# ShijieZhou-UCLA/feature-3dgs

Hardware: NVIDIA H100
Metric: views/sec fwd+bwd @1M Gaussians/1080p/feat_dim=128 (higher is better)
Workload: dtype f32

## Files before the change

### feature-3dgs_b200/csrc/composite_common.cuh

```cuda
#pragma once
#include <initializer_list>

#include "kernels.h"

namespace f3dgs {

constexpr int kBlocksPerTile = 8;
constexpr int kProducerWarp = 0;
constexpr int kAlphaWarp0 = 4;
constexpr int kAlphaWarps = kBlocksPerTile;
constexpr int kFeatWarp0 = kAlphaWarp0 + kAlphaWarps;
constexpr int kRegsProducer = 40;
constexpr int kStageEntries = 32;
constexpr int kStages = 6;
constexpr int kWSlots = 2;
constexpr int kDoneSlots = 8;

template <int CH, typename TF = float>
struct alignas(128) Stage {
    TF feat[CH > 0 ? kStageEntries : 1][CH > 0 ? CH : 4];
    float4 rec0[kStageEntries];
    float4 rec1[kStageEntries];
    float4 rec2[kStageEntries];
    uint32_t listpos[kStageEntries];
    uint32_t gid[kStageEntries];
    uint32_t n;
    uint32_t last;
    uint32_t first;
    int32_t work;
    uint32_t done_slot;
};

struct alignas(128) WSlot {
    float w[kStageEntries][32];
    uint32_t pm[kStageEntries];
    uint32_t km;
    uint32_t last;
    uint32_t first;
    int32_t work;
};

template <int CH, typename TF = float, int WB = kBlocksPerTile, int WJ = kWSlots>
struct alignas(128) RingV2 {
    using Feat = TF;
    static constexpr int kWB = WB, kWJ = WJ;
    Stage<CH, TF> stage[kStages];
    WSlot ws[WB][WJ];
    uint64_t full[kStages];
    uint64_t empty[kStages];
    uint64_t listed[kStages];
    uint64_t wfull[WB][WJ];
    uint64_t wempty[WB][WJ];
    uint32_t done_mask[kDoneSlots];
};

using RingSlim = RingV2<0, float, 1, 1>;

static_assert(sizeof(RingV2<0>) == 81664 && sizeof(RingSlim) == 16128, "ring layout changed");
static_assert(sizeof(RingV2<32>) == 106240 && sizeof(RingV2<64>) == 130816 && sizeof(RingV2<128>) == 179968,
              "ring layout changed");
static_assert(sizeof(RingV2<32, __half>) == 93952 && sizeof(RingV2<64, __half>) == 106240 &&
                  sizeof(RingV2<128, __half>) == 130816,
              "ring layout changed");

__device__ __forceinline__ int block_x0(int tile_x, int b) { return tile_x * 16 + (b & 1) * 8; }
__device__ __forceinline__ int block_y0(int tile_y, int b) { return tile_y * 16 + (b >> 1) * 4; }
__device__ __forceinline__ int slot_px(int p) { return ((p >> 2) & 3) * 2 + (p & 1); }
__device__ __forceinline__ int slot_py(int p) { return (p >> 4) * 2 + ((p >> 1) & 1); }

template <int NQ>
__device__ __forceinline__ float& tile_px(float2 (&t)[NQ][2][4], int qi, int i, int c) {
    return (i & 1) ? t[qi][i >> 1][c].y : t[qi][i >> 1][c].x;
}
template <int NQ>
__device__ __forceinline__ float& tile_run_px(float2 (&t)[NQ][2][4], int y, int half, int k, int c) {
    return tile_px(t, ((y >> 1) * 4 + half * 2 + (k >> 1)) % NQ, (y & 1) * 2 + (k & 1), c);
}
template <int NQ>
__device__ __forceinline__ float4 tile_run(float2 (&t)[NQ][2][4], int y, int half, int c) {
    return make_float4(tile_run_px(t, y, half, 0, c), tile_run_px(t, y, half, 1, c), tile_run_px(t, y, half, 2, c),
                       tile_run_px(t, y, half, 3, c));
}
template <int NQ>
__device__ __forceinline__ void set_tile_run(float2 (&t)[NQ][2][4], int y, int half, int c, float4 v) {
    tile_run_px(t, y, half, 0, c) = v.x;
    tile_run_px(t, y, half, 1, c) = v.y;
    tile_run_px(t, y, half, 2, c) = v.z;
    tile_run_px(t, y, half, 3, c) = v.w;
}

template <int G, int NQ, typename T, class Row, class Run, class Px>
__device__ __forceinline__ void for_tile_pixels(T* plane, int bx0, int by0, int W, int H, int grp, bool rows, bool runs,
                                                Row row, Run run, Px px) {
    if (G == 1 && rows && bx0 + 8 <= W) {
#pragma unroll
        for (int y = 0; y < 4; y++) {
            const int yy = by0 + y;
            if (yy >= H) continue;
            row(plane + (size_t)yy * W + bx0, y);
        }
    } else if (G == 1 && runs) {
#pragma unroll
        for (int y = 0; y < 4; y++) {
            const int yy = by0 + y;
            if (yy >= H) continue;
#pragma unroll
            for (int half = 0; half < 2; half++) {
                const int xx = bx0 + half * 4;
                if (xx >= W) continue;
                run(plane + (size_t)yy * W + xx, y, half);
            }
        }
    } else {
#pragma unroll
        for (int qi = 0; qi < NQ; qi++) {
            const int q = qi * G + grp;
#pragma unroll
            for (int i = 0; i < 4; i++) {
                const int xx = bx0 + (q & 3) * 2 + (i & 1), yy = by0 + (q >> 2) * 2 + (i >> 1);
                if (xx < W && yy < H) px(plane + (size_t)yy * W + xx, qi, i);
            }
        }
    }
}

__device__ __forceinline__ float4 to_float4(float4 v) { return v; }
__device__ __forceinline__ float4 to_float4(uint2 v) {
    const float2 a = __half22float2(*reinterpret_cast<const __half2*>(&v.x));
    const float2 b = __half22float2(*reinterpret_cast<const __half2*>(&v.y));
    return make_float4(a.x, a.y, b.x, b.y);
}

__device__ __forceinline__ size_t list_begin(uint32_t begin, uint32_t end, int b) {
    return kBlocksPerTile * (size_t)begin + (size_t)b * (end - begin);
}

struct SplatAlpha {
    float dx, dy, G, alpha;
};
__device__ __forceinline__ SplatAlpha splat_alpha(const float4 r0, const float4 r1, float pxf, float pyf, bool valid) {
    SplatAlpha s;
    s.dx = r0.x - pxf;
    s.dy = r0.y - pyf;
    const float power = -0.5f * (r1.x * s.dx * s.dx + r1.z * s.dy * s.dy) - r1.y * s.dx * s.dy;
    s.G = expf(power);
    const float av = fminf(0.99f, r1.w * s.G);
    s.alpha = (valid && !(power > 0.0f) && !(av < 1.0f / 255.0f)) ? av : 0.f;
    return s;
}

__device__ __forceinline__ bool footprint_hits_rect(const float4 r0, const float4 r1, float x0, float x1, float y0,
                                                    float y1) {
    const bool box = (r0.x + r0.z >= x0) && (r0.x - r0.z <= x1) && (r0.y + r0.w >= y0) && (r0.y - r0.w <= y1);
    if (!box) return false;
    const float dxl = r0.x - x1, dxh = r0.x - x0, dyl = r0.y - y1, dyh = r0.y - y0;
    if (r0.z > 1.0e30f || (dxl <= 0.f && dxh >= 0.f && dyl <= 0.f && dyh >= 0.f)) return true;
    const float a = r1.x, b = r1.y, c = r1.z;
    const float tau = 2.02f * __logf(255.0f * r1.w) + 0.02f;
    const float nb_ia = -b * rcp_approx(a), nb_ic = -b * rcp_approx(c);
    float q = 3.0e38f;
#pragma unroll
    for (int k = 0; k < 2; k++) {
        const float ex_ = k ? dxh : dxl;
        const float ty = fminf(fmaxf(nb_ic * ex_, dyl), dyh);
        q = fminf(q, a * ex_ * ex_ + (2.f * b * ex_ + c * ty) * ty);
        const float ey_ = k ? dyh : dyl;
        const float tx = fminf(fmaxf(nb_ia * ey_, dxl), dxh);
        q = fminf(q, c * ey_ * ey_ + (2.f * b * ey_ + a * tx) * tx);
    }
    return q <= tau;
}

template <int N>
__device__ __forceinline__ void reg_dec() {
    asm volatile("setmaxnreg.dec.sync.aligned.u32 %0;" ::"n"(N));
}
template <int N>
__device__ __forceinline__ void reg_inc() {
    asm volatile("setmaxnreg.inc.sync.aligned.u32 %0;" ::"n"(N));
}

template <int CH, typename RING>
__device__ __forceinline__ void ring_init(RING& ring, int n_stage_consumers, int n_full_arrivals = 1) {
    if (threadIdx.x == 0) {
        for (int s = 0; s < kStages; s++) {
            mbar_init(&ring.full[s], n_full_arrivals);
            mbar_init(&ring.empty[s], n_stage_consumers);
            mbar_init(&ring.listed[s], 1);
        }
        for (int b = 0; b < RING::kWB; b++)
            for (int j = 0; j < RING::kWJ; j++) {
                mbar_init(&ring.wfull[b][j], 1);
                mbar_init(&ring.wempty[b][j], 1);
            }
        for (int i = 0; i < kDoneSlots; i++) ring.done_mask[i] = 0;
        mbar_fence_init();
    }
    if (CH > 0) {
        float4* p = reinterpret_cast<float4*>(&ring.stage[0]);
        const int n16 = (int)(sizeof(ring.stage) / 16);
        for (int i = threadIdx.x; i < n16; i += blockDim.x) p[i] = make_float4(0.f, 0.f, 0.f, 0.f);
        asm volatile("fence.proxy.async.shared::cta;" ::: "memory");
    }
}

struct ProducerArgs {
    const uint2* ranges;
    const uint32_t* point_list;
    const SplatRec* rec;
    const void* features;
    const uint32_t* n_contrib;
    int* work_counter;
    int W, H, C;
    int tiles_x, num_tiles, chunks;
    int use_bulk;
};

inline ProducerArgs producer_args(const ViewParams& vp, const uint2* ranges, const uint32_t* point_list,
                                  const SplatRec* rec, const uint32_t* n_contrib, int* work_counter) {
    return ProducerArgs{ranges, point_list, rec, nullptr, n_contrib, work_counter, vp.W, vp.H, 0, (int)vp.grid_x,
                        (int)(vp.grid_x * vp.grid_y), 1, 0};
}

inline int channel_chunk(int C) { return C <= 32 ? 32 : (C <= 64 ? 64 : 128); }

template <auto... K>
cudaError_t device_sms(int& sms, size_t smem) {
    static std::atomic<int> sms_of_device[64];
    int dev = 0;
    cudaGetDevice(&dev);
    if (dev < 0 || dev >= 64) return cudaErrorInvalidDevice;
    if (sms_of_device[dev].load() == 0) {
        for (const void* k : std::initializer_list<const void*>{reinterpret_cast<const void*>(K)...}) {
            const cudaError_t e = cudaFuncSetAttribute(k, cudaFuncAttributeMaxDynamicSharedMemorySize, (int)smem);
            if (e != cudaSuccess) return e;
        }
        int n = 0;
        cudaDeviceGetAttribute(&n, cudaDevAttrMultiProcessorCount, dev);
        sms_of_device[dev].store(n > 0 ? n : 132);
    }
    sms = sms_of_device[dev].load();
    return cudaSuccess;
}

template <int CH, bool REVERSE, typename RING = RingV2<CH>>
__device__ __forceinline__ void producer_loop(RING& ring, const ProducerArgs& pa) {
    using TF = typename RING::Feat;
    constexpr bool COPYWARP = CH > 0;
    const int lane = threadIdx.x & 31;
    int s = 0;
    uint32_t empty_parity = 1;
    mbar_wait(&ring.empty[0], empty_parity);

    uint32_t seq = 0;
    auto publish = [&](uint32_t n, uint32_t last, uint32_t first, int work) {
        __syncwarp();
        if (lane == 0) {
            Stage<CH, TF>& st = ring.stage[s];
            st.done_slot = seq % kDoneSlots;
            st.n = n;
            st.last = last;
            st.first = first;
            st.work = work;
            mbar_arrive(&ring.full[s]);
            if (COPYWARP) mbar_arrive(&ring.listed[s]);
        }
        __syncwarp();
    };
    auto advance = [&]() {
        s++;
        if (s == kStages) {
            s = 0;
            empty_parity ^= 1;
        }
        mbar_wait_sleep(&ring.empty[s], empty_parity, 64);
    };

    const int num_work = pa.num_tiles * pa.chunks;
    int pending = 0;
    if (lane == 0) pending = atomicAdd(pa.work_counter, 1);
    for (;;) {
        const int work = __shfl_sync(0xffffffffu, pending, 0);
        if (lane == 0 && work < num_work) pending = atomicAdd(pa.work_counter, 1);
        if (work >= num_work) {
            publish(0, 1, 1, -1);
            break;
        }
        const int tile = work / pa.chunks, chunk = work - tile * pa.chunks;
        const int tile_x = tile % pa.tiles_x, tile_y = tile / pa.tiles_x;
        const uint2 range = pa.ranges[tile];
        const uint32_t range_begin = range.x;
        uint32_t walk_count = range.y - range.x;
        if (REVERSE) {
            uint32_t tmax = 0;
            const int yy = tile_y * 16 + (lane >> 1), xb = tile_x * 16 + (lane & 1) * 8;
            if (yy < pa.H)
                for (int i = 0; i < 8; i++)
                    if (xb + i < pa.W) tmax = max(tmax, pa.n_contrib[(size_t)yy * pa.W + xb + i]);
#pragma unroll
            for (int o = 16; o > 0; o >>= 1) tmax = max(tmax, __shfl_xor_sync(0xffffffffu, tmax, o));
            walk_count = min(walk_count, tmax);
        }
        const float tx0 = (float)(tile_x * 16), ty0 = (float)(tile_y * 16), tx1 = tx0 + 15.f, ty1 = ty0 + 15.f;
        const int chunk_off = chunk * CH;
        const int row_floats = (CH > 0 && pa.features != nullptr) ? min(CH, pa.C - chunk_off) : 0;
        seq++;
        uint32_t* done = &ring.done_mask[seq % kDoneSlots];
        if (lane == 0) *reinterpret_cast<volatile uint32_t*>(done) = 0;
        __syncwarp();

        auto list_index = [&](uint32_t i) -> uint32_t {
            return REVERSE ? (range_begin + walk_count - 1 - i) : (range_begin + i);
        };
        auto store_entry = [&](uint32_t slot, uint32_t gid, uint32_t lpos, float4 r0, float4 r1, float4 r2) {
            Stage<CH, TF>& st = ring.stage[s];
            st.rec0[slot] = r0;
            st.rec1[slot] = r1;
            st.rec2[slot] = r2;
            st.listpos[slot] = lpos;
            st.gid[slot] = gid;
            if (CH > 0 && row_floats > 0) {
                const TF* src = static_cast<const TF*>(pa.features) + (size_t)gid * pa.C + chunk_off;
                if (!pa.use_bulk)
                    for (int c = 0; c < row_floats; c++) st.feat[slot][c] = __ldg(src + c);
            }
        };

        uint32_t fill = 0, first = 1;
        const uint32_t nchunks = (walk_count + 31) / 32;
        uint32_t id_cur = 0, id_nxt = 0;
        float4 a0, a1, a2;
        a0 = a1 = a2 = make_float4(0.f, 0.f, 0.f, 0.f);
        if (nchunks > 0) {
            if (lane < walk_count) id_cur = pa.point_list[list_index(lane)];
            if (32 + lane < walk_count) id_nxt = pa.point_list[list_index(32 + lane)];
            if (lane < walk_count) {
                const float4* r = reinterpret_cast<const float4*>(pa.rec + id_cur);
                a0 = __ldg(r); a1 = __ldg(r + 1); a2 = __ldg(r + 2);
            }
        }
        for (uint32_t c = 0; c < nchunks; c++) {
            if (*reinterpret_cast<volatile uint32_t*>(done) == (1u << kBlocksPerTile) - 1u) break;
            float4 b0, b1, b2;
            b0 = b1 = b2 = make_float4(0.f, 0.f, 0.f, 0.f);
            const uint32_t i1 = (c + 1) * 32 + lane, i2 = (c + 2) * 32 + lane;
            uint32_t id_nn = 0;
            if (i1 < walk_count) {
                const float4* r = reinterpret_cast<const float4*>(pa.rec + id_nxt);
                b0 = __ldg(r); b1 = __ldg(r + 1); b2 = __ldg(r + 2);
            }
            if (i2 < walk_count) id_nn = pa.point_list[list_index(i2)];

            const uint32_t i0 = c * 32 + lane;
            const bool valid = i0 < walk_count;
            const bool keep = valid && footprint_hits_rect(a0, a1, tx0, tx1, ty0, ty1);
            const uint32_t m = __ballot_sync(0xffffffffu, keep);
            const uint32_t cnt = __popc(m);
            const uint32_t rank = __popc(m & ((1u << lane) - 1u));
            const uint32_t lpos = list_index(i0) - range_begin + 1;
            const uint32_t room = kStageEntries - fill;
            if (keep && rank < room) store_entry(fill + rank, id_cur, lpos, a0, a1, a2);
            if (cnt >= room) {
                publish(kStageEntries, 0, first, work);
                first = 0;
                advance();
                if (keep && rank >= room) store_entry(rank - room, id_cur, lpos, a0, a1, a2);
                fill = cnt - room;
            } else {
                fill += cnt;
            }
            a0 = b0; a1 = b1; a2 = b2;
            id_cur = id_nxt;
            id_nxt = id_nn;
        }
        publish(fill, 1, first, work);
        advance();
    }
}

template <int CH, typename TF>
__device__ __forceinline__ void copy_loop(RingV2<CH, TF>& ring, const ProducerArgs& pa) {
    const int lane = threadIdx.x & 31;
    int s = 0;
    uint32_t parity = 0;
    for (;;) {
        mbar_wait(&ring.listed[s], parity);
        Stage<CH, TF>& st = ring.stage[s];
        const uint32_t n = st.n;
        const int work = st.work;
        if (work < 0) {
            if (lane == 0) mbar_arrive(&ring.full[s]);
            break;
        }
        const int chunk_off = (work % pa.chunks) * CH;
        const uint32_t row_bytes = (uint32_t)min(CH, pa.C - chunk_off) * (uint32_t)sizeof(TF);
        if (pa.use_bulk && n > 0) {
            if (lane == 0) mbar_arrive_expect_tx(&ring.full[s], n * row_bytes);
            __syncwarp();
            if (lane < n)
                bulk_g2s(&st.feat[lane][0],
                         static_cast<const TF*>(pa.features) + (size_t)st.gid[lane] * pa.C + chunk_off, row_bytes,
                         &ring.full[s]);
        } else {
            if (lane == 0) mbar_arrive(&ring.full[s]);
        }
        if (++s == kStages) {
            s = 0;
            parity ^= 1;
        }
    }
}

}
```

### feature-3dgs_b200/csrc/composite_fwd.cu

```cuda
#include <type_traits>

#include "composite_common.cuh"

namespace f3dgs {

constexpr int kFwdThreads = (kFeatWarp0 + kBlocksPerTile) * 32;
constexpr int kRegsAlpha = 64;
constexpr int kRegsFeature = 152;

template <typename TF>
struct FwdArgs {
    ProducerArgs pa;
    const float* bg;
    float* final_T;
    uint32_t* n_contrib;
    float* out_color;
    TF* out_feature;
    float* out_depth;
    int vec_store;
};

template <typename TF>
using Feat4 = std::conditional_t<std::is_same_v<TF, float>, float4, uint2>;
__device__ __forceinline__ uint32_t pack_half2(float a, float b) {
    const __half2 h = __floats2half2_rn(a, b);
    return *reinterpret_cast<const uint32_t*>(&h);
}
__device__ __forceinline__ void st_row(float* p, float4 a, float4 b) { st_na_f8(p, a, b); }
__device__ __forceinline__ void st_row(__half* p, float4 a, float4 b) {
    st_na_b128(p, make_uint4(pack_half2(a.x, a.y), pack_half2(a.z, a.w), pack_half2(b.x, b.y), pack_half2(b.z, b.w)));
}
__device__ __forceinline__ void st_run(float* p, float4 v) { st_na_f4(p, v); }
__device__ __forceinline__ void st_run(__half* p, float4 v) {
    st_na_b64(p, make_uint2(pack_half2(v.x, v.y), pack_half2(v.z, v.w)));
}
__device__ __forceinline__ void st_px(float* p, float v) { *p = v; }
__device__ __forceinline__ void st_px(__half* p, float v) { *p = __float2half_rn(v); }

template <int CH, typename TF>
__global__ void __launch_bounds__(kFwdThreads, 1)
composite_fwd_kernel(const FwdArgs<TF> args) {
    extern __shared__ __align__(128) unsigned char smem_raw[];
    using RING = RingV2<CH, TF>;
    RING& ring = *reinterpret_cast<RING*>(smem_raw);
    const int warp = __shfl_sync(0xffffffffu, threadIdx.x >> 5, 0);
    const int lane = threadIdx.x & 31;
    const int W = args.pa.W, H = args.pa.H, C = args.pa.C;
    const size_t HW = (size_t)H * W;

    ring_init<CH>(ring, CH > 0 ? kAlphaWarps + kBlocksPerTile : kAlphaWarps, CH > 0 ? 2 : 1);
    __syncthreads();

    if (warp < kAlphaWarp0) {
        reg_dec<kRegsProducer>();
        if (warp == kProducerWarp) {
            producer_loop<CH, false>(ring, args.pa);
        } else if constexpr (CH > 0) {
            if (warp == kProducerWarp + 1) copy_loop<CH, TF>(ring, args.pa);
        }
        return;
    }

    if (warp < kFeatWarp0) {
        reg_dec<kRegsAlpha>();
        const int b = warp - kAlphaWarp0;
        int s = 0, j = 0;
        uint32_t parity = 0, wparity = 1;
        float T = 1.f, Cr = 0.f, Cg = 0.f, Cb = 0.f, Dp = 0.f, pxf = 0.f, pyf = 0.f, fbx0 = 0.f, fby0 = 0.f;
        uint32_t last_contrib = 0;
        int px = 0, py = 0, chunk = 0;
        bool done = true, inside = false, blk_done = true;
        for (;;) {
            mbar_wait(&ring.full[s], parity);
            Stage<CH, TF>& st = ring.stage[s];
            const uint32_t n = st.n, last = st.last, first = st.first;
            const int work = st.work;
            if (work < 0) break;
            if (first) {
                const int tile = work / args.pa.chunks;
                chunk = work - tile * args.pa.chunks;
                const int tile_x = tile % args.pa.tiles_x, tile_y = tile / args.pa.tiles_x;
                const int bx0 = block_x0(tile_x, b), by0 = block_y0(tile_y, b);
                px = bx0 + slot_px(lane);
                py = by0 + slot_py(lane);
                inside = px < W && py < H;
                pxf = (float)px; pyf = (float)py;
                fbx0 = (float)bx0; fby0 = (float)by0;
                T = 1.f; Cr = Cg = Cb = Dp = 0.f;
                last_contrib = 0;
                done = !inside;
                blk_done = __all_sync(0xffffffffu, done);
                if (blk_done && lane == 0) atomicOr(&ring.done_mask[st.done_slot], 1u << b);
            }
            WSlot* ws = &ring.ws[b][j];
            if (CH > 0) mbar_wait(&ring.wempty[b][j], wparity);
            uint32_t km = 0;
            if (!blk_done && n > 0) {
                bool hit = false;
                if (lane < n) hit = footprint_hits_rect(st.rec0[lane], st.rec1[lane], fbx0, fbx0 + 7.f, fby0, fby0 + 3.f);
                uint32_t am = __ballot_sync(0xffffffffu, hit);
                while (am) {
                    int kk[4];
                    bool vk[4];
                    float al[4];
#pragma unroll
                    for (int u = 0; u < 4; u++) {
                        vk[u] = am != 0;
                        kk[u] = vk[u] ? (__ffs(am) - 1) : 0;
                        am &= am - 1;
                    }
#pragma unroll
                    for (int u = 0; u < 4; u++) al[u] = splat_alpha(st.rec0[kk[u]], st.rec1[kk[u]], pxf, pyf, vk[u]).alpha;
#pragma unroll
                    for (int u = 0; u < 4; u++) {
                        if (!vk[u]) break;
                        const float4 r2 = st.rec2[kk[u]];
                        const uint32_t lp = st.listpos[kk[u]];
                        const float alpha = al[u];
                        const float test_T = T * (1 - alpha);
                        const bool act = !done && alpha > 0.f;
                        const bool stop = act && (test_T < 0.0001f);
                        const bool blend = act && !stop;
                        done = done || stop;
                        const float wgt = blend ? alpha * T : 0.f;
                        const float nCr = Cr + r2.x * alpha * T;
                        const float nCg = Cg + r2.y * alpha * T;
                        const float nCb = Cb + r2.z * alpha * T;
                        const float nDp = Dp + r2.w * (alpha * T);
                        Cr = blend ? nCr : Cr;
                        Cg = blend ? nCg : Cg;
                        Cb = blend ? nCb : Cb;
                        Dp = blend ? nDp : Dp;
                        T = blend ? test_T : T;
                        last_contrib = blend ? lp : last_contrib;
                        const uint32_t pm = __ballot_sync(0xffffffffu, blend);
                        if (CH > 0) {
                            ws->w[kk[u]][lane] = wgt;
                            if (lane == 0) ws->pm[kk[u]] = pm;
                            km |= (pm ? 1u : 0u) << kk[u];
                        }
                    }
                }
                if (__all_sync(0xffffffffu, done)) {
                    blk_done = true;
                    if (lane == 0) atomicOr(&ring.done_mask[st.done_slot], 1u << b);
                }
            }
            if (CH > 0) {
                __syncwarp();
                if (lane == 0) {
                    ws->km = km;
                    ws->last = last;
                    ws->first = first;
                    ws->work = work;
                    mbar_arrive(&ring.wfull[b][j]);
                }
            }
            __syncwarp();
            if (lane == 0) mbar_arrive(&ring.empty[s]);
            if (last && chunk == 0 && inside) {
                const size_t pix = (size_t)py * W + px;
                args.final_T[pix] = T;
                args.n_contrib[pix] = last_contrib;
                args.out_color[pix] = Cr + T * args.bg[0];
                args.out_color[HW + pix] = Cg + T * args.bg[1];
                args.out_color[2 * HW + pix] = Cb + T * args.bg[2];
                args.out_depth[pix] = Dp;
            }
            if (++s == kStages) { s = 0; parity ^= 1; }
            if (CH > 0 && ++j == kWSlots) { j = 0; wparity ^= 1; }
        }
        if (CH > 0) {
            mbar_wait(&ring.wempty[b][j], wparity);
            if (lane == 0) {
                ring.ws[b][j].work = -1;
                ring.ws[b][j].km = 0;
                mbar_arrive(&ring.wfull[b][j]);
            }
        }
        return;
    }

    if (CH == 0) return;
    reg_inc<kRegsFeature>();
    {
        constexpr int LPR = CH > 0 ? CH / 4 : 32;
        constexpr int G = 32 / LPR;
        constexpr int NQ = 8 / G;
        const int b = warp - kFeatWarp0;
        const int grp = lane / LPR, cl = lane % LPR;
        float2 acc2[NQ][2][4];
#pragma unroll
        for (int q = 0; q < NQ; q++)
#pragma unroll
            for (int i = 0; i < 4; i++)
#pragma unroll
                for (int c = 0; c < 4; c++) tile_px(acc2, q, i, c) = 0.f;
#define FEAT_ROW_FMA(Q, ROW, W2)                                                                     \
        do {                                                                                             \
            const float2 w2_ = (W2);                                                                     \
            const float fr_[4] = {f.x, f.y, f.z, f.w};                                                   \
            _Pragma("unroll") for (int c_ = 0; c_ < 4; c_++)                                             \
                acc2[Q][ROW][c_] = fma2_rn(make_float2(fr_[c_], fr_[c_]), w2_, acc2[Q][ROW][c_]);     \
        } while (0)
        int s = 0, j = 0;
        uint32_t parity = 0, wparity = 0;
        for (;;) {
            mbar_wait(&ring.wfull[b][j], wparity);
            const WSlot& ws = ring.ws[b][j];
            const int work = ws.work;
            if (work < 0) break;
            uint32_t km = ws.km;
            const uint32_t last = ws.last;
            mbar_wait(&ring.full[s], parity);
            const Stage<CH, TF>& st = ring.stage[s];
            int kn = km ? __ffs(km) - 1 : 0;
            uint32_t pm_n = ws.pm[kn];
            Feat4<TF> f_n = *reinterpret_cast<const Feat4<TF>*>(&st.feat[kn][cl * 4]);
            while (km) {
                const int k = kn;
                const uint32_t pm = pm_n;
                const float4 f = to_float4(f_n);
                km &= km - 1;
                kn = km ? __ffs(km) - 1 : k;
                pm_n = ws.pm[kn];
                f_n = *reinterpret_cast<const Feat4<TF>*>(&st.feat[kn][cl * 4]);
#pragma unroll
                for (int qi = 0; qi < NQ; qi++) {
                    const int q = qi * G + grp;
                    if ((pm >> (4 * q)) & 0xFu) {
                        const float4 w4 = *reinterpret_cast<const float4*>(&ws.w[k][4 * q]);
                        if ((pm >> (4 * q)) & 0x3u) FEAT_ROW_FMA(qi, 0, make_float2(w4.x, w4.y));
                        if ((pm >> (4 * q)) & 0xCu) FEAT_ROW_FMA(qi, 1, make_float2(w4.z, w4.w));
                    }
                }
            }
            __syncwarp();
            if (lane == 0) {
                mbar_arrive(&ring.wempty[b][j]);
                mbar_arrive(&ring.empty[s]);
            }
            if (last) {
                const int tile = work / args.pa.chunks, chunk = work - tile * args.pa.chunks;
                const int tile_x = tile % args.pa.tiles_x, tile_y = tile / args.pa.tiles_x;
                const int bx0 = block_x0(tile_x, b), by0 = block_y0(tile_y, b);
#pragma unroll
                for (int c = 0; c < 4; c++) {
                    const int ch = chunk * CH + cl * 4 + c;
                    if (ch < C)
                        for_tile_pixels<G, NQ>(
                            args.out_feature + (size_t)ch * HW, bx0, by0, W, H, grp, args.vec_store & 2,
                            args.vec_store & 1,
                            [&](TF* p, int y) { st_row(p, tile_run(acc2, y, 0, c), tile_run(acc2, y, 1, c)); },
                            [&](TF* p, int y, int half) { st_run(p, tile_run(acc2, y, half, c)); },
                            [&](TF* p, int qi, int i) { st_px(p, tile_px(acc2, qi, i, c)); });
                }
#pragma unroll
                for (int q = 0; q < NQ; q++)
#pragma unroll
                    for (int i = 0; i < 4; i++)
#pragma unroll
                        for (int c = 0; c < 4; c++) tile_px(acc2, q, i, c) = 0.f;
            }
            if (++s == kStages) { s = 0; parity ^= 1; }
            if (++j == kWSlots) { j = 0; wparity ^= 1; }
        }
    }
#undef FEAT_ROW_FMA
}

template <int CH, typename TF>
static cudaError_t launch_fwd_t(const ViewParams& vp, const uint2* ranges, const uint32_t* point_list,
                                const SplatRec* rec, const TF* features, const float* bg, float* final_T,
                                uint32_t* n_contrib, float* out_color, TF* out_feature, float* out_depth,
                                int* work_counter, cudaStream_t s) {
    const size_t smem = sizeof(RingV2<CH, TF>);
    int num_sms = 0;
    cudaError_t e = device_sms<composite_fwd_kernel<CH, TF>>(num_sms, smem);
    if (e != cudaSuccess) return e;
    FwdArgs<TF> a;
    a.pa = producer_args(vp, ranges, point_list, rec, nullptr, work_counter);
    a.pa.features = CH > 0 ? features : nullptr;
    a.pa.C = vp.C;
    a.pa.chunks = CH > 0 ? (vp.C + CH - 1) / CH : 1;
    constexpr int kPer16 = 16 / (int)sizeof(TF);
    a.pa.use_bulk = (CH > 0 && vp.C % kPer16 == 0 && (reinterpret_cast<uintptr_t>(features) & 15) == 0) ? 1 : 0;
    a.bg = bg; a.final_T = final_T; a.n_contrib = n_contrib;
    a.out_color = out_color; a.out_feature = out_feature; a.out_depth = out_depth;
    const uintptr_t out_addr = reinterpret_cast<uintptr_t>(out_feature);
    a.vec_store = (vp.W % 4 == 0 && (out_addr & (4 * sizeof(TF) - 1)) == 0) ? 1 : 0;
    if (vp.W % 8 == 0 && (out_addr & (8 * sizeof(TF) - 1)) == 0) a.vec_store |= 2;
    e = cudaMemsetAsync(work_counter, 0, sizeof(int), s);
    if (e != cudaSuccess) return e;
    const int grid = min(a.pa.num_tiles * a.pa.chunks, num_sms);
    composite_fwd_kernel<CH, TF><<<grid, kFwdThreads, smem, s>>>(a);
    g_launches++;
    return cudaGetLastError();
}

template <typename TF>
cudaError_t launch_composite_fwd(const ViewParams& vp, const uint2* ranges, const uint32_t* point_list,
                                 const SplatRec* rec, const TF* features, const float* bg,
                                 float* final_T, uint32_t* n_contrib, float* out_color,
                                 TF* out_feature, float* out_depth, int* work_counter, cudaStream_t s) {
    if (vp.C == 0)
        return launch_fwd_t<0, float>(vp, ranges, point_list, rec, nullptr, bg, final_T, n_contrib, out_color, nullptr,
                                      out_depth, work_counter, s);
    const int ch = channel_chunk(vp.C);
    const auto launch = ch == 32 ? launch_fwd_t<32, TF> : ch == 64 ? launch_fwd_t<64, TF> : launch_fwd_t<128, TF>;
    return launch(vp, ranges, point_list, rec, features, bg, final_T, n_contrib, out_color, out_feature, out_depth,
                  work_counter, s);
}

template cudaError_t launch_composite_fwd<float>(const ViewParams&, const uint2*, const uint32_t*, const SplatRec*,
                                                 const float*, const float*, float*, uint32_t*, float*, float*, float*,
                                                 int*, cudaStream_t);
template cudaError_t launch_composite_fwd<__half>(const ViewParams&, const uint2*, const uint32_t*, const SplatRec*,
                                                  const __half*, const float*, float*, uint32_t*, float*, __half*,
                                                  float*, int*, cudaStream_t);

}
```

Baseline: 142.2.

## Split each feature-accumulation block across two warps by pixel-row halves

Doubles the feature consumer warps per tile block so each warp handles two of the four pixel rows, with separate per-half contribution masks and a weight-slot empty barrier expecting two arrivals. This halves each feature warp's register tile, so the feature register budget drops and alpha warps get fewer registers, aiming for more latency hiding and less skipped work per half. In exchange it adds more warps sharing shared-memory bandwidth, duplicate feature loads from the stage by both halves, and extra barrier arrivals.

```diff
diff --git a/feature-3dgs_b200/csrc/composite_common.cuh b/feature-3dgs_b200/csrc/composite_common.cuh
--- a/feature-3dgs_b200/csrc/composite_common.cuh
+++ b/feature-3dgs_b200/csrc/composite_common.cuh
@@ -34,11 +34,12 @@
 struct alignas(128) WSlot {
     float w[kStageEntries][32];
     uint32_t pm[kStageEntries];
-    uint32_t km;
+    uint32_t km[2];
     uint32_t last;
     uint32_t first;
     int32_t work;
 };
+static_assert(sizeof(WSlot) == 4352, "weight slot layout changed");
 
 template <int CH, typename TF = float, int WB = kBlocksPerTile, int WJ = kWSlots>
 struct alignas(128) RingV2 {
@@ -89,19 +90,20 @@
     tile_run_px(t, y, half, 3, c) = v.w;
 }
 
-template <int G, int NQ, typename T, class Row, class Run, class Px>
+template <int G, int NQ, int NY = 4, typename T, class Row, class Run, class Px>
 __device__ __forceinline__ void for_tile_pixels(T* plane, int bx0, int by0, int W, int H, int grp, bool rows, bool runs,
                                                 Row row, Run run, Px px) {
+    static_assert(NQ * G * 2 == NY * 4, "a register tile of NQ quads per lane group covers NY rows of 8 pixels");
     if (G == 1 && rows && bx0 + 8 <= W) {
 #pragma unroll
-        for (int y = 0; y < 4; y++) {
+        for (int y = 0; y < NY; y++) {
             const int yy = by0 + y;
             if (yy >= H) continue;
             row(plane + (size_t)yy * W + bx0, y);
         }
     } else if (G == 1 && runs) {
 #pragma unroll
-        for (int y = 0; y < 4; y++) {
+        for (int y = 0; y < NY; y++) {
             const int yy = by0 + y;
             if (yy >= H) continue;
 #pragma unroll
@@ -181,7 +183,8 @@
 }
 
 template <int CH, typename RING>
-__device__ __forceinline__ void ring_init(RING& ring, int n_stage_consumers, int n_full_arrivals = 1) {
+__device__ __forceinline__ void ring_init(RING& ring, int n_stage_consumers, int n_full_arrivals = 1,
+                                          int n_wslot_consumers = 1) {
     if (threadIdx.x == 0) {
         for (int s = 0; s < kStages; s++) {
             mbar_init(&ring.full[s], n_full_arrivals);
@@ -191,7 +194,7 @@
         for (int b = 0; b < RING::kWB; b++)
             for (int j = 0; j < RING::kWJ; j++) {
                 mbar_init(&ring.wfull[b][j], 1);
-                mbar_init(&ring.wempty[b][j], 1);
+                mbar_init(&ring.wempty[b][j], n_wslot_consumers);
             }
         for (int i = 0; i < kDoneSlots; i++) ring.done_mask[i] = 0;
         mbar_fence_init();
diff --git a/feature-3dgs_b200/csrc/composite_fwd.cu b/feature-3dgs_b200/csrc/composite_fwd.cu
--- a/feature-3dgs_b200/csrc/composite_fwd.cu
+++ b/feature-3dgs_b200/csrc/composite_fwd.cu
@@ -4,9 +4,11 @@
 
 namespace f3dgs {
 
-constexpr int kFwdThreads = (kFeatWarp0 + kBlocksPerTile) * 32;
-constexpr int kRegsAlpha = 64;
-constexpr int kRegsFeature = 152;
+template <int CH>
+constexpr int kFwdThreads = (kFeatWarp0 + (CH > 0 ? 2 : 1) * kBlocksPerTile) * 32;
+template <int CH>
+constexpr int kRegsAlpha = CH > 0 ? 56 : 64;
+constexpr int kRegsFeature = 88;
 
 template <typename TF>
 struct FwdArgs {
@@ -38,7 +40,7 @@
 __device__ __forceinline__ void st_px(__half* p, float v) { *p = __float2half_rn(v); }
 
 template <int CH, typename TF>
-__global__ void __launch_bounds__(kFwdThreads, 1)
+__global__ void __launch_bounds__(kFwdThreads<CH>, 1)
 composite_fwd_kernel(const FwdArgs<TF> args) {
     extern __shared__ __align__(128) unsigned char smem_raw[];
     using RING = RingV2<CH, TF>;
@@ -48,7 +50,7 @@
     const int W = args.pa.W, H = args.pa.H, C = args.pa.C;
     const size_t HW = (size_t)H * W;
 
-    ring_init<CH>(ring, CH > 0 ? kAlphaWarps + kBlocksPerTile : kAlphaWarps, CH > 0 ? 2 : 1);
+    ring_init<CH>(ring, CH > 0 ? kAlphaWarps + 2 * kBlocksPerTile : kAlphaWarps, CH > 0 ? 2 : 1, CH > 0 ? 2 : 1);
     __syncthreads();
 
     if (warp < kAlphaWarp0) {
@@ -62,7 +64,7 @@
     }
 
     if (warp < kFeatWarp0) {
-        reg_dec<kRegsAlpha>();
+        reg_dec<kRegsAlpha<CH>>();
         const int b = warp - kAlphaWarp0;
         int s = 0, j = 0;
         uint32_t parity = 0, wparity = 1;
@@ -94,7 +96,7 @@
             }
             WSlot* ws = &ring.ws[b][j];
             if (CH > 0) mbar_wait(&ring.wempty[b][j], wparity);
-            uint32_t km = 0;
+            uint32_t km0 = 0, km1 = 0;
             if (!blk_done && n > 0) {
                 bool hit = false;
                 if (lane < n) hit = footprint_hits_rect(st.rec0[lane], st.rec1[lane], fbx0, fbx0 + 7.f, fby0, fby0 + 3.f);
@@ -137,7 +139,8 @@
                         if (CH > 0) {
                             ws->w[kk[u]][lane] = wgt;
                             if (lane == 0) ws->pm[kk[u]] = pm;
-                            km |= (pm ? 1u : 0u) << kk[u];
+                            km0 |= ((pm & 0xFFFFu) ? 1u : 0u) << kk[u];
+                            km1 |= ((pm >> 16) ? 1u : 0u) << kk[u];
                         }
                     }
                 }
@@ -149,7 +152,8 @@
             if (CH > 0) {
                 __syncwarp();
                 if (lane == 0) {
-                    ws->km = km;
+                    ws->km[0] = km0;
+                    ws->km[1] = km1;
                     ws->last = last;
                     ws->first = first;
                     ws->work = work;
@@ -174,7 +178,7 @@
             mbar_wait(&ring.wempty[b][j], wparity);
             if (lane == 0) {
                 ring.ws[b][j].work = -1;
-                ring.ws[b][j].km = 0;
+                ring.ws[b][j].km[0] = ring.ws[b][j].km[1] = 0;
                 mbar_arrive(&ring.wfull[b][j]);
             }
         }
@@ -186,8 +190,8 @@
     {
         constexpr int LPR = CH > 0 ? CH / 4 : 32;
         constexpr int G = 32 / LPR;
-        constexpr int NQ = 8 / G;
-        const int b = warp - kFeatWarp0;
+        constexpr int NQ = 4 / G;
+        const int b = (warp - kFeatWarp0) >> 1, h = (warp - kFeatWarp0) & 1;
         const int grp = lane / LPR, cl = lane % LPR;
         float2 acc2[NQ][2][4];
 #pragma unroll
@@ -210,7 +214,7 @@
             const WSlot& ws = ring.ws[b][j];
             const int work = ws.work;
             if (work < 0) break;
-            uint32_t km = ws.km;
+            uint32_t km = ws.km[h];
             const uint32_t last = ws.last;
             mbar_wait(&ring.full[s], parity);
             const Stage<CH, TF>& st = ring.stage[s];
@@ -219,7 +223,7 @@
             Feat4<TF> f_n = *reinterpret_cast<const Feat4<TF>*>(&st.feat[kn][cl * 4]);
             while (km) {
                 const int k = kn;
-                const uint32_t pm = pm_n;
+                const uint32_t pm = pm_n >> (16 * h);
                 const float4 f = to_float4(f_n);
                 km &= km - 1;
                 kn = km ? __ffs(km) - 1 : k;
@@ -229,7 +233,7 @@
                 for (int qi = 0; qi < NQ; qi++) {
                     const int q = qi * G + grp;
                     if ((pm >> (4 * q)) & 0xFu) {
-                        const float4 w4 = *reinterpret_cast<const float4*>(&ws.w[k][4 * q]);
+                        const float4 w4 = *reinterpret_cast<const float4*>(&ws.w[k][16 * h + 4 * q]);
                         if ((pm >> (4 * q)) & 0x3u) FEAT_ROW_FMA(qi, 0, make_float2(w4.x, w4.y));
                         if ((pm >> (4 * q)) & 0xCu) FEAT_ROW_FMA(qi, 1, make_float2(w4.z, w4.w));
                     }
@@ -243,12 +247,12 @@
             if (last) {
                 const int tile = work / args.pa.chunks, chunk = work - tile * args.pa.chunks;
                 const int tile_x = tile % args.pa.tiles_x, tile_y = tile / args.pa.tiles_x;
-                const int bx0 = block_x0(tile_x, b), by0 = block_y0(tile_y, b);
+                const int bx0 = block_x0(tile_x, b), by0 = block_y0(tile_y, b) + 2 * h;
 #pragma unroll
                 for (int c = 0; c < 4; c++) {
                     const int ch = chunk * CH + cl * 4 + c;
                     if (ch < C)
-                        for_tile_pixels<G, NQ>(
+                        for_tile_pixels<G, NQ, 2>(
                             args.out_feature + (size_t)ch * HW, bx0, by0, W, H, grp, args.vec_store & 2,
                             args.vec_store & 1,
                             [&](TF* p, int y) { st_row(p, tile_run(acc2, y, 0, c), tile_run(acc2, y, 1, c)); },
@@ -293,7 +297,7 @@
     e = cudaMemsetAsync(work_counter, 0, sizeof(int), s);
     if (e != cudaSuccess) return e;
     const int grid = min(a.pa.num_tiles * a.pa.chunks, num_sms);
-    composite_fwd_kernel<CH, TF><<<grid, kFwdThreads, smem, s>>>(a);
+    composite_fwd_kernel<CH, TF><<<grid, kFwdThreads<CH>, smem, s>>>(a);
     g_launches++;
     return cudaGetLastError();
 }
```

After: 150.0, median of 6. 1.06x the previous value.
